# plindhorst/Ray-Tracing-Project

Measured on AMD Instinct MI355X. Metric: Mrays/s (primary) + frame ms at 1920x1080, 1M-tri BVH, 1/2/4/8 GPU, higher is better.
Workload: dtype f32; 1 GPU; C3: 1000000 random triangles (SplitMix64 seed 12345), 1920x1080 primary rays, eye (0,0,1), 1 light; frame=1920x1080, triangles=1000000, mode=primary, parallelism=tiles/1 (one GPU, whole frame), launcher=none, frames_in_flight=4, prewarm_frames=200, hw_queues=4, bvh_nodes=1145398, bvh_depth=26, ref_boxes=4480, builder=sbvh-gpu

## Files before the change

### ray-tracing-project_amd/csrc/rt_device.hip

```cpp
#include <errno.h>
#include <fcntl.h>
#include <signal.h>
#include <sys/file.h>
#include <unistd.h>

#include <atomic>
#include <cctype>
#include <chrono>
#include <condition_variable>
#include <memory>
#include <mutex>
#include <string>
#include <thread>
#include <vector>

#include "rt_dispatch.h"
#include "rt_kernels.h"

namespace rt {

constexpr int kLptBuckets = 32, kLptThreads = 512, kLptRefresh = 8;
constexpr bool kLptMoved = true;
constexpr int kLptDilate = 2;
constexpr bool kLptPred = true;
// ... 1154 lines not shown
  rt_scene::FrameSlot& slot = s->slots[slot_id];
  if ((rc = ensure_fb(slot, (size_t)fr->width * fr->height))) return rc;
  hipStream_t st = (hipStream_t)slot.stream;
  FrameParams P;
  fill_scene_params(s, P);
  fill_camera_lights(P, cam, lights, n_lights);
  P.W = fr->width, P.H = fr->height, P.tiles_x = (fr->width + 15) / 16, P.tiles_y = (fr->height + 15) / 16;
  P.shard_index = si, P.shard_count = sc, P.super_tile = frame_super_tile(sc);
  P.mode = fr->mode, P.flags = fr->flags, P.shadows = fr->mode == RT_MODE_FULL ? 1 : 0;
  P.rgb = slot.d_rgb, P.face_out = slot.d_face, P.t_out = slot.d_t, P.hits = slot.d_hits;
  P.stats = s->d_stats, P.face_boxcolor = s->d_face_boxcolor;
  if (fr->flags & RT_FRAME_STATS) {
    for (int k = 0; k < s->n_slots; k++)
      if (k != slot_id && s->slots[k].last_done) HIPCHECK(hipStreamWaitEvent(st, (hipEvent_t)s->slots[k].last_done, 0));
    HIPCHECK(hipMemsetAsync(s->d_stats, 0, kStatSlots * sizeof(unsigned long long), st));
  }
  FrameInputs in;
  in.mode = fr->mode, in.max_depth = fr->max_depth, in.flags = fr->flags;
  in.tiles_x = P.tiles_x, in.tiles_y = P.tiles_y, in.shard_index = si, in.shard_count = sc;
  in.variant = kernel_variant(), in.has_wide4 = P.sc.n_nodes4 > 0;
  in.record_bytes = (uint64_t)(s->hs.nodes.size() + s->hs.tris.size()) * 64;
  for (int k = 0; k < s->n_slots; k++)
    if (k != slot_id && s->slots[k].last_done && hipEventQuery((hipEvent_t)s->slots[k].last_done) == hipErrorNotReady)
      in.alone = false;
  in.split_k = knob_int("RT_SPLIT_K", kSplitK, 0, INT_MAX);
  in.split_kp = knob_int("RT_SPLIT_KP", kSplitKPrimary, 0, INT_MAX);
  in.timeline_split = knob_int("RT_TIMELINE_SPLIT", kKnobUnset, INT_MIN, INT_MAX) != kKnobUnset;
  const FramePlan plan = plan_frame(in);
  P.n_tiles_shard = plan.grid;
  P.max_depth = plan.depth;
  if (plan.primary_binary_tree) P.sc.wide_copy_bytes = 0;
  if (fr->flags & RT_FRAME_TIMELINE) {
    const size_t waves = in.timeline_split ? 2 * plan.units : plan.units;
    if ((rc = ensure_wave_records(slot.d_timeline, slot.timeline_waves, waves, st))) return rc;
    P.timeline = slot.d_timeline;
    s->last_timeline_waves = (int64_t)waves;
  }
  if ((fr->flags & RT_FRAME_STATS) && (fr->flags & RT_FRAME_WAVE_STATS)) {
    if (!plan.writes_wave_stats) {
      set_error("rt_render: RT_FRAME_WAVE_STATS needs the mode's own max_depth (the generic-depth kernel keeps no per-wave counts)");
      return RT_ERR_UNSUPPORTED;
    }
    const size_t lw = (size_t)plan.grid * 4;
    if ((rc = ensure_wave_records(slot.d_wave_stats, slot.wave_stats_waves, lw, st))) return rc;
    P.wave_stats = slot.d_wave_stats;
    s->last_wave_stats_waves = (int64_t)lw;
  }
  if (plan.pipeline_buffers) {
    if (sc > 1) { set_error("rt_render: the FULL stage-pipeline variant renders whole frames only"); return RT_ERR_UNSUPPORTED; }
    if ((rc = ensure_full(slot, (size_t)P.tiles_x * 16 * (size_t)P.tiles_y * 16))) return rc;
    bind_full(slot, P);
  }
  P.xcd_remap = plan.xcd_remap;
  if (plan.rotate_bands) P.xcd_rot = (int32_t)(s->band_rot++ & 7u);
  if (plan.needs_variants && !variants_linked()) {
    set_error("rt_render: kernel variant %d is an A/B build option, not in this library (make variants)", in.variant);
    return RT_ERR_UNSUPPORTED;
  }
  bool lpt_sort = false, lpt_dilated = false;
  if (plan.lpt && (rc = lpt_begin(s, plan, cam, st, P, lpt_sort, lpt_dilated))) return rc;
  if (s->ev_used + 3 > s->ev_pool.size()) {
    if (s->ev_pool.size() >= 3 * 2048) { set_error("more than 2048 renders without rt_synchronize"); return RT_ERR_INVALID; }
    for (int k = 0; k < 3; k++) {
      hipEvent_t e;
      HIPCHECK(hipEventCreate(&e));
      s->ev_pool.push_back(e);
    }
  }
  hipEvent_t* ev = (hipEvent_t*)&s->ev_pool[s->ev_used];
  s->ev_used += 3;
  HIPCHECK(hipEventRecord(ev[0], st));
  if ((rc = launch_frame(plan, s, slot, P, st, ev[1]))) return rc;
  if (lpt_sort && (rc = lpt_end(s, plan, st, lpt_dilated))) return rc;
  HIPCHECK(hipEventRecord(ev[2], st));
  slot.last_done = ev[2];
  note_frame(s, slot_id, fr, P);
  return RT_OK;
}

static int check_prefetch_word(rt_scene* s) {
#ifdef RT_CHECK_PREFETCH
  uint32_t w = 0;
  HIPCHECK(hipMemcpy(&w, s->d_pf_check, 4, hipMemcpyDeviceToHost));
  if (w) {
    set_error("RT_CHECK_PREFETCH: out-of-range scalar load offset (sites 0x%x: 0 node, 1/2 child prefetch, 3 leaf "
              "prefetch, 4 wide prefetch, 5 wide node)", w);
    return RT_ERR_HIP;
  }
#endif
  (void)s;
  return RT_OK;
}

static int sync_one(rt_scene* s, rt_stats* out) {
  int rc = check_device_scene(s);
  if (rc) return rc;
  for (int k = 0; k < s->n_slots; k++) HIPCHECK(hipStreamSynchronize((hipStream_t)s->slots[k].stream));
  if ((rc = check_prefetch_word(s))) return rc;
  struct Reset {
    rt_scene* s;
    ~Reset() {
      s->ev_used = 0;
      s->pending = false;
      for (int k = 0; k < s->n_slots; k++) s->slots[k].last_done = nullptr;
    }
  } reset_{s};
// ... 771 lines not shown
```

### ray-tracing-project_amd/csrc/rt_internal.h

```cpp
#pragma once
#include <cstdint>
#if defined(__HIPCC__) || defined(__HIP__)
#include <hip/hip_runtime.h>
#else
struct uint2 { unsigned int x, y; };
#endif

#include "rt_math.h"

namespace rt {

constexpr uint32_t kLeafBit = 0x80000000u;
constexpr uint32_t kLeafCountShift = 27;
constexpr uint32_t kLeafFirstMask = (1u << 27) - 1;
constexpr int kMaxLeaf = 16;
constexpr uint32_t kMaxFaces = (1u << 25) - 1;
constexpr int kMaxDepth = 60;
constexpr uint32_t kSafeNormalBit = 0x80000000u;
constexpr uint32_t kBoxCertBit = 0x40000000u;
constexpr uint32_t kBoxIndexMask = 0x3FFFFFFFu;

inline uint64_t record_layout(uint64_t n_nodes, uint64_t n_tris, uint64_t n_wide, uint64_t* wide_base) {
  const uint64_t bytes = (n_nodes + n_tris) * 64;
  *wide_base = 0;
  if (bytes > 0xFFFFFFFFull) return 0;
  const uint64_t wb = (bytes + 127) & ~(uint64_t)127, wide_bytes = 8 * n_wide * 128;
  if (n_wide == 0 || wb + wide_bytes > (uint64_t)kLeafBit) return bytes;
  *wide_base = wb;
  return wb + wide_bytes;
}

enum { TRAV_B2_VGPR = 0, TRAV_B2_LDS = 1, TRAV_W4 = 2, TRAV_LANE = 3 };

enum VariantBit : int {
  VB_VGPR_STACK = 1,
  VB_WIDE4 = 2,
  VB_XCD_ORDER = 4,
  VB_FULL_PIPELINE = 16,
  VB_PIPE_LANE_REFL = 32,
  VB_PIPE_LANE_SHADOW1 = 64,
  VB_PIPE_LANE_SHADOW0 = 128,
  VB_TWO_RAYS_PER_LANE = 256,
  VB_XCD_RUNS_4 = 512,
  VB_XCD_RUNS_16 = 1024,
  VB_DISPATCH_ORDER = 1536,
  VB_PERSISTENT = 2048,
  VB_PERSISTENT_NO_STEAL = 4096,
  VB_FULL_8_WAVES = 8192,
  VB_FULL_SMALL_BUILD = 16384,
  VB_SPLIT_PRIMARY = 32768,
  VB_GENERIC_DEPTH = 65536,
  VB_NO_LPT = 131072,
  VB_COARSE_COST_BUCKETS = 262144,
  VB_LPT_IN_FLIGHT = 524288,
  VB_DUAL_CHAIN = 1048576,
  VB_PRIMARY_BINARY_TREE = 2097152,
  VB_PRIMARY_UNFUSED = VB_SPLIT_PRIMARY | VB_TWO_RAYS_PER_LANE | VB_PERSISTENT,
  VB_DUAL_EXCLUDED = VB_VGPR_STACK | VB_WIDE4 | VB_XCD_ORDER | VB_PRIMARY_UNFUSED | VB_GENERIC_DEPTH,
};

// ... 105 lines not shown
};

struct FrameParams {
  DevScene sc;
  float Minv[16];
  float MS[9];
  DevMat defmat;
  float bg[3];
  float vinv[16];
  float eye[3];
  float eye_obj[3];
  float vp[4];
  float xscale, yscale;
  int32_t n_lights;
  Light lights[32];
  int32_t W, H, tiles_x, tiles_y;
  int32_t xcd_remap;
  int32_t xcd_rot;
  int32_t shard_index, shard_count, n_tiles_shard;
  int32_t super_tile;
  int32_t mode, flags;
  int32_t max_depth;
  int32_t shadows;
  float* rgb;
  int32_t* face_out;
  float* t_out;
  unsigned long long* stats;
  uint2* hits;
  HitState* state0;
  HitState* state1;
  RayRec* refl;
  uint2* hits1;
  uint32_t* blk0;
  uint32_t* blk1;
  uint32_t* list0;
  uint32_t* list1;
  uint32_t* wcount0;
  uint32_t* wcount1;
  uint32_t* woff0;
  uint32_t* woff1;
  uint32_t* counters;
  int32_t n_waves_max;
  uint32_t* timeline;
  const uint32_t* order;
  uint32_t* cost;
  uint32_t* cost_dil;
  int32_t dil_r;
  int32_t pred;
  float pred_proj[4];
  float pred_step[3];
  uint32_t* wave_stats;
  int32_t split_k;
  const float* face_boxcolor;
};

struct RayParams {
  const float* o;
  const float* d;
  int32_t n;
  int32_t* face;
  float* t;
  float* P;
  int32_t* blocked;
  float* N;
  float* rgb;
};

}
```

### ray-tracing-project_amd/csrc/rt_kernels.h

```cpp
#pragma once
#include <hip/hip_runtime.h>

#include <algorithm>
#include <atomic>
#include <cmath>
#include <cstddef>
#include <cstdio>
#include <cstring>
#include <type_traits>
#include <vector>

#include "rt_kat.h"
#include "rt_scene.h"

using rt::f3;

#define HIPCHECK(expr)                                                                   \
  do {                                                                                   \
    hipError_t e_ = (expr);                                                              \
    if (e_ != hipSuccess) {                                                              \
      rt::set_error("%s failed: %s (%s:%d)", #expr, hipGetErrorString(e_), __FILE__, __LINE__); \
      return RT_ERR_HIP;                                                                 \
    }                                                                                    \
  } while (0)
// ... 91 lines not shown
  const float dm = fmaxf(fmaxf(fabsf(r.d.x), fabsf(r.d.y)), fabsf(r.d.z));
  const bool certified = om <= kCullOriginMax && dm >= kCullDirMin && dm <= kCullDirMax;
  if (certified) {
    r.id = f3{__builtin_amdgcn_rcpf(nudge(r.d.x)), __builtin_amdgcn_rcpf(nudge(r.d.y)),
              __builtin_amdgcn_rcpf(nudge(r.d.z))};
    const float pr = kCullPadRel * om;
    const float p = pr > static_pad ? pr : 0.0f;
    r.oa = f3{-(r.o.x + p) * r.id.x, -(r.o.y + p) * r.id.y, -(r.o.z + p) * r.id.z};
    r.ob = f3{-(r.o.x - p) * r.id.x, -(r.o.y - p) * r.id.y, -(r.o.z - p) * r.id.z};
  } else {
    r.id = f3{copysignf(1.0f, nudge(r.d.x)), copysignf(1.0f, nudge(r.d.y)), copysignf(1.0f, nudge(r.d.z))};
    r.oa = f3{-r.id.x * INFINITY, -r.id.y * INFINITY, -r.id.z * INFINITY};
    r.ob = f3{r.id.x * INFINITY, r.id.y * INFINITY, r.id.z * INFINITY};
  }
}

struct Span {
  float tmin, tmax;
};
__device__ __forceinline__ Span slab(float lx, float hx, float ly, float hy, float lz, float hz, const Ray& r,
                                     float tmax_ray) {
  const float tx0 = __builtin_fmaf(lx, r.id.x, r.oa.x), tx1 = __builtin_fmaf(hx, r.id.x, r.ob.x);
  const float ty0 = __builtin_fmaf(ly, r.id.y, r.oa.y), ty1 = __builtin_fmaf(hy, r.id.y, r.ob.y);
  const float tz0 = __builtin_fmaf(lz, r.id.z, r.oa.z), tz1 = __builtin_fmaf(hz, r.id.z, r.ob.z);
  Span s;
  s.tmin = fmaxf(fmaxf(fminf(tx0, tx1), fminf(ty0, ty1)), fmaxf(fminf(tz0, tz1), 0.0f));
  s.tmax = fminf(fminf(fmaxf(tx0, tx1), fmaxf(ty0, ty1)), fminf(fmaxf(tz0, tz1), tmax_ray));
  return s;
}
template <int OCT>
__device__ __forceinline__ Span slab_o(float lx, float hx, float ly, float hy, float lz, float hz, const Ray& r,
                                       float tmax_ray) {
  if (OCT < 0) return slab(lx, hx, ly, hy, lz, hz, r, tmax_ray);
  const float nx = (OCT & 1) ? hx : lx, fx = (OCT & 1) ? lx : hx;
  const float ny = (OCT & 2) ? hy : ly, fy = (OCT & 2) ? ly : hy;
  const float nz = (OCT & 4) ? hz : lz, fz = (OCT & 4) ? lz : hz;
  const float nox = (OCT & 1) ? r.ob.x : r.oa.x, fox = (OCT & 1) ? r.oa.x : r.ob.x;
  const float noy = (OCT & 2) ? r.ob.y : r.oa.y, foy = (OCT & 2) ? r.oa.y : r.ob.y;
  const float noz = (OCT & 4) ? r.ob.z : r.oa.z, foz = (OCT & 4) ? r.oa.z : r.ob.z;
  Span s;
  s.tmin = fmaxf(fmaxf(__builtin_fmaf(nx, r.id.x, nox), __builtin_fmaf(ny, r.id.y, noy)),
                 fmaxf(__builtin_fmaf(nz, r.id.z, noz), 0.0f));
  asm("v_min3_f32 %0, %1, %2, %3\n\tv_min_f32 %0, %0, %4"
      : "=&v"(s.tmax)
      : "v"(__builtin_fmaf(fx, r.id.x, fox)), "v"(__builtin_fmaf(fy, r.id.y, foy)),
        "v"(__builtin_fmaf(fz, r.id.z, foz)), "v"(tmax_ray));
  return s;
}
constexpr int kFcmpOLE = 5;
__device__ __forceinline__ uint64_t mask_le(float a, float b) { return __builtin_amdgcn_fcmpf(a, b, kFcmpOLE); }

__device__ __forceinline__ bool ref_box_test(const DevScene& S, const Ray& r, const float* bx) {
  const float MS[9] = {S.Minv[0], S.Minv[1], S.Minv[2], S.Minv[4], S.Minv[5], S.Minv[6], S.Minv[8], S.Minv[9], S.Minv[10]};
  const f3 dd = normalized(m3v3(MS, r.d));
  const float lo[3] = {bx[0], bx[1], bx[2]}, hi[3] = {bx[4], bx[5], bx[6]};
  const float o2[3] = {r.o2.x, r.o2.y, r.o2.z}, d2[3] = {dd.x, dd.y, dd.z};
  float tin3[3], tout3[3];
#pragma unroll
  for (int k = 0; k < 3; k++) {
    const float a = (lo[k] - o2[k]) / d2[k];
    const float b = (hi[k] - o2[k]) / d2[k];
    tin3[k] = smin(a, b);
    tout3[k] = smax(a, b);
  }
  const float tin = smax(tin3[0], smax(tin3[1], tin3[2]));
  const float tout = smin(tout3[0], smin(tout3[1], tout3[2]));
  return !(tin > tout || tout < 0);
}

__device__ __forceinline__ f3 ld3(const float* p) { return f3{p[0], p[1], p[2]}; }

constexpr int kFcmpOEQ = 1, kFcmpOGE = 3, kFcmpOLT = 4, kFcmpUNE = 14, kIcmpULT = 36;
template <int PRED>
__device__ __forceinline__ uint64_t fmask(float a, float b) { return __builtin_amdgcn_fcmpf(a, b, PRED); }
__device__ __forceinline__ bool lane_in(uint64_t m) { return __builtin_amdgcn_inverse_ballot_w64(m); }

__device__ __forceinline__ uint64_t accept_candidate(const DevScene& P, const TriRec64& tr, uint32_t slot, f3 e0, f3 e2,
                                                    f3 a0, f3 a1, f3 a2, f3 p, const Ray& r, uint64_t cand) {
  if (!(tr.box & kSafeNormalBit)) {
    const float area0 = norm(a0) / 2, area1 = norm(a1) / 2, area2 = norm(a2) / 2;
    const float area = norm(cross(e0, neg(e2))) / 2;
    const float* fs = P.fshade + 12 * (size_t)slot;
    const f3 n0 = ld3(fs), n1 = ld3(fs + 4), n2 = ld3(fs + 8);
    const f3 nn = blend_normal(n0, n1, n2, area0, area1, area2, area);
    cand &= fmask<kFcmpUNE>(norm(nn), 0.0f);
  }
  if (tr.box & kBoxCertBit) {
    const float om = fmaxf(fmaxf(fabsf(r.o2.x), fabsf(r.o2.y)), fabsf(r.o2.z));
    if ((cand & ~ballot(om <= P.cert_origin_max)) == 0) return cand;
  }
  const float* bx = P.refbox + 8 * (size_t)(tr.box & kBoxIndexMask);
  const f3 X = affv3(P.Minv, p);
  const float lo[3] = {bx[0], bx[1], bx[2]}, hi[3] = {bx[4], bx[5], bx[6]};
  const float xs[3] = {X.x, X.y, X.z}, os[3] = {r.o2.x, r.o2.y, r.o2.z};
  bool inside = true;
#pragma unroll
  for (int k = 0; k < 3; k++) {
    const float m = 1e-5f * ((hi[k] - lo[k]) + fabsf(lo[k]) + fabsf(hi[k]) + fabsf(os[k])) + 1e-30f;
    inside = inside & (xs[k] > lo[k] + m) & (xs[k] < hi[k] - m);
  }
  const uint64_t ins = ballot(inside);
  if ((cand & ~ins) == 0) return cand;
  return cand & (ins | ballot(ref_box_test(P, r, bx)));
}

template <bool ANY, bool STATS = false>
__device__ __forceinline__ void test_tri(const DevScene& P, const TriRec64& tr, uint32_t slot, const Ray& r,
// ... 561 lines not shown
        switch (oct) {
          RT_WIDE_CASE(0) RT_WIDE_CASE(1) RT_WIDE_CASE(2) RT_WIDE_CASE(3)
          RT_WIDE_CASE(4) RT_WIDE_CASE(5) RT_WIDE_CASE(6) default: RT_WIDE_CASE(7)
        }
#undef RT_WIDE_CASE
      }
      if (!STATS && SL) {
        switch (oct) {
          case 0: traverse_fast<ANY, 0>(P, r, active, h, found, L.stack[wv]); return;
          case 1: traverse_fast<ANY, 1>(P, r, active, h, found, L.stack[wv]); return;
          case 2: traverse_fast<ANY, 2>(P, r, active, h, found, L.stack[wv]); return;
          case 3: traverse_fast<ANY, 3>(P, r, active, h, found, L.stack[wv]); return;
          case 4: traverse_fast<ANY, 4>(P, r, active, h, found, L.stack[wv]); return;
          case 5: traverse_fast<ANY, 5>(P, r, active, h, found, L.stack[wv]); return;
          case 6: traverse_fast<ANY, 6>(P, r, active, h, found, L.stack[wv]); return;
          default: traverse_fast<ANY, 7>(P, r, active, h, found, L.stack[wv]); return;
        }
      }
      switch (oct) {
        case 0: traverse<ANY, STATS, SL, 0>(P, r, active, h, found, L.stack[wv], cnt); return;
        case 1: traverse<ANY, STATS, SL, 1>(P, r, active, h, found, L.stack[wv], cnt); return;
        case 2: traverse<ANY, STATS, SL, 2>(P, r, active, h, found, L.stack[wv], cnt); return;
        case 3: traverse<ANY, STATS, SL, 3>(P, r, active, h, found, L.stack[wv], cnt); return;
        case 4: traverse<ANY, STATS, SL, 4>(P, r, active, h, found, L.stack[wv], cnt); return;
        case 5: traverse<ANY, STATS, SL, 5>(P, r, active, h, found, L.stack[wv], cnt); return;
        case 6: traverse<ANY, STATS, SL, 6>(P, r, active, h, found, L.stack[wv], cnt); return;
        default: traverse<ANY, STATS, SL, 7>(P, r, active, h, found, L.stack[wv], cnt); return;
      }
    }
  }
  trace<ANY, STATS, TRAV>(P, r, active, h, found, L, wv, cnt);
}
template <bool STATS, int TRAV, bool WIDE = false>
__device__ __forceinline__ void trace_closest_oct(const DevScene& P, const Ray& r, bool active, Hit& h,
                                                  WaveLds<TRAV, STATS>& L, int wv, uint32_t* cnt) {
  bool found = false;
  trace_oct<false, STATS, TRAV, WIDE, false>(P, r, active, h, found, L, wv, cnt);
}
template <bool ANY, bool STATS, int TRAV>
__device__ __forceinline__ void trace_full_ray(const DevScene& P, const Ray& r, bool active, Hit& h, bool& found,
                                               WaveLds<TRAV, STATS>& L, int wv, uint32_t* cnt) {
  trace<ANY, STATS, TRAV>(P, r, active, h, found, L, wv, cnt);
}

struct MatState {
  f3 ka, kd, ks;
  float ns;
};

__device__ __forceinline__ MatState load_mat(const DevMat& m) {
  return MatState{f3{m.ka[0], m.ka[1], m.ka[2]}, f3{m.kd[0], m.kd[1], m.kd[2]}, f3{m.ks[0], m.ks[1], m.ks[2]}, m.ns};
}

__device__ __forceinline__ f3 hit_normal(const DevScene& P, const TriRec64& tr, uint32_t slot, f3 p, int32_t& mat) {
  const f3 n{tr.nx, tr.ny, tr.nz};
  const f3 w0{tr.w0x, tr.w0y, tr.w0z}, w1{tr.w1x, tr.w1y, tr.w1z}, w2{tr.w2x, tr.w2y, tr.w2z};
  const f3 e0 = sub(w1, w0), e1 = sub(w2, w1), e2 = sub(w0, w2);
  const f3 a0 = cross(e0, sub(p, w0)), a1 = cross(e1, sub(p, w1)), a2 = cross(e2, sub(p, w2));
  const float4* fs = reinterpret_cast<const float4*>(P.fshade + 12 * (size_t)slot);
  const float4 n0 = fs[0];
  mat = __float_as_int(n0.w);
  if (dot(n, a0) < 0 || dot(n, a1) < 0 || dot(n, a2) < 0) return f3{0.0f, 0.0f, 0.0f};
  const float area0 = norm(a0) / 2, area1 = norm(a1) / 2, area2 = norm(a2) / 2;
  const float area = norm(cross(e0, neg(e2))) / 2;
  const float4 n1 = fs[1], n2 = fs[2];
  return blend_normal(f3{n0.x, n0.y, n0.z}, f3{n1.x, n1.y, n1.z}, f3{n2.x, n2.y, n2.z}, area0, area1, area2, area);
}

__device__ __forceinline__ TriRec64 vload_tri(const TriRec64* base, uint32_t i) {
  const float4* p = reinterpret_cast<const float4*>(base + i);
  TriRec64 r;
  float4* q = reinterpret_cast<float4*>(&r);
  q[0] = p[0]; q[1] = p[1]; q[2] = p[2]; q[3] = p[3];
  return r;
}


__device__ __forceinline__ Light frame_light(int l) {
  typedef const __attribute__((address_space(4))) char* KArg;
  typedef const __attribute__((address_space(4))) Light* KLight;
  const KArg base = (KArg)__builtin_amdgcn_kernarg_segment_ptr();
  const KLight q = (KLight)(base + offsetof(FrameParams, lights) + (size_t)l * sizeof(Light));
  Light r;
  for (int k = 0; k < 3; k++) {
    r.p[k] = q->p[k];
    r.c[k] = q->c[k];
  }
  r.kind = q->kind;
  return r;
}

__device__ __forceinline__ f3 light_dir(f3 p, const Light& l) {
  if (l.kind == RT_LIGHT_DIRECTIONAL) return f3{l.p[0], l.p[1], l.p[2]};
  return neg(normalized(sub(p, f3{l.p[0], l.p[1], l.p[2]})));
}

struct HitInfo {
  f3 p, n;
  int32_t mat;
  uint32_t face;
};

__device__ __forceinline__ f3 phong(const FrameParams& P, MatState& st, const HitInfo& hi, f3 o, f3 L, const float* I) {
  if (hi.mat != -1) st = load_mat(P.sc.mats[hi.mat]);
  const f3 R = phong_r(L, hi.n);
  const f3 E = normalized(sub(o, hi.p));
  const float dif = smax(dot(L, hi.n), 0.0f);
  const float spe = smax(pow_ref(dot(R, E), st.ns), 0.0f);
  return f3{(I[0] * st.ka.x + (I[0] * st.kd.x) * dif) + (I[0] * st.ks.x) * spe,
            (I[1] * st.ka.y + (I[1] * st.kd.y) * dif) + (I[1] * st.ks.y) * spe,
            (I[2] * st.ka.z + (I[2] * st.kd.z) * dif) + (I[2] * st.ks.z) * spe};
}

__device__ __forceinline__ float clamp01(float x) { return smax(smin(x, 1.0f), 0.0f); }

template <bool SHADOWS, bool STATS, int TRAV, bool OCTSH = false, bool SPLIT = false>
__device__ __forceinline__ f3 calc_color(const FrameParams& P, MatState& st, const HitInfo& hi, f3 o, bool lane_hit,
                                         WaveLds<TRAV, STATS>* lds, int wv, uint32_t* cnt) {
  f3 sum{0.0f, 0.0f, 0.0f};
  for (int l = 0; l < P.n_lights; l++) {
    const Light lt = frame_light(l);
    const f3 L = light_dir(hi.p, lt);
    bool blocked = false;
    if (SHADOWS) {
      Ray sr;
      sr.o = offset(hi.p, L, 0.003f);
      sr.d = L;
      sr.o2 = affv3(P.Minv, hi.p);
      setup_cull(sr, P.sc.static_pad);
      Hit hh{INFINITY, 0xFFFFFFFFu, 0xFFFFFFFFu};
      if (STATS && lane_hit) cnt[ST_TOTAL]++;
      if (OCTSH)
        trace_oct<true, STATS, TRAV, false, SPLIT>(P.sc, sr, lane_hit, hh, blocked, *lds, wv, cnt);
      else trace_full_ray<true, STATS, TRAV>(P.sc, sr, lane_hit, hh, blocked, *lds, wv, cnt);
    }
    f3 c{0.0f, 0.0f, 0.0f};
    if (lane_hit && !blocked) c = phong(P, st, hi, o, L, lt.c);
    sum = f3{sum.x + c.x, sum.y + c.y, sum.z + c.z};
  }
  return f3{clamp01(sum.x), clamp01(sum.y), clamp01(sum.z)};
}

struct PixelCoord {
  int px, py, wv, lane;
  int slot;
  int qw;
  int sub;
  bool active;
};

template <int WPB = 4>
__device__ __forceinline__ PixelCoord pixel_coord(const FrameParams& P) {
  PixelCoord c;
  c.lane = threadIdx.x & 63;
  int nb, b;
  int bid = (int)blockIdx.x;
  c.sub = -1;
  if (WPB == 1 && P.order != nullptr) {
    const uint32_t k = (uint32_t)P.split_k, nlog = gridDim.x - 3u * k;
    uint32_t pos = blockIdx.x;
    if (k > 0) {
      if (pos < 4u * k) {
        c.sub = (int)(pos & 3u);
        pos >>= 2;
      } else {
        pos -= 3u * k;
      }
    }
    const uint32_t o = uniform(P.order[pos]);
    bid = o < nlog ? (int)o : (int)pos;
  } else if (P.xcd_remap >= 2) {
    const int C = P.xcd_remap, G = 8 * C, full = ((int)gridDim.x / G) * G;
    if (bid < full) {
      const int x = ((bid & 7) + P.xcd_rot) & 7, k = bid >> 3;
      bid = (k / C) * G + x * C + (k % C);
    }
  }
  if (WPB == 4) {
    c.wv = (int)uniform(threadIdx.x >> 6);
    c.slot = c.wv;
    nb = (int)gridDim.x;
    b = bid;
  } else {
    c.wv = bid & 3;
    c.slot = 0;
    nb = (int)((gridDim.x - 3u * (uint32_t)P.split_k) >> 2);
    b = bid >> 2;
  }
  c.qw = b * 4 + c.wv;
  int L = b;
  if (P.xcd_remap == 1) {
    const int q = nb >> 3, rr = nb & 7, x = b & 7, k = b >> 3;
    L = x < rr ? x * (q + 1) + k : rr * (q + 1) + (x - rr) * q + k;
  }
  int tx, ty;
  shard_tile_xy(P.tiles_x, P.super_tile, P.shard_index, P.shard_count, L, tx, ty);
  c.px = tx * 16 + (c.wv & 1) * 8 + (c.lane & 7);
  c.py = ty * 16 + (c.wv >> 1) * 8 + (c.lane >> 3);
  c.active = c.px < P.W && c.py < P.H && (c.sub < 0 || (c.lane >> 4) == c.sub);
  return c;
}

__device__ __forceinline__ Ray primary_ray(const FrameParams& P, int px, int py) {
  Ray r;
  const float nx = (float)(2.0 * (double)((float)px - P.vp[0]) / (double)P.vp[2] - 1.0);
  const float ny = (float)(1.0 - 2.0 * (double)((float)py - P.vp[1]) / (double)P.vp[3]);
  const f3 w = affv3(P.vinv, f3{nx * P.xscale, ny * P.yscale, -1.0f});
  r.o = f3{P.eye[0], P.eye[1], P.eye[2]};
  r.d = normalized(sub(w, r.o));
  r.o2 = f3{P.eye_obj[0], P.eye_obj[1], P.eye_obj[2]};
  setup_cull(r, P.sc.static_pad);
  return r;
}

template <typename T>
__device__ __forceinline__ T late_kernarg(size_t off) {
  uint32_t o = (uint32_t)off;
  asm volatile("" : "+s"(o));
  typedef const __attribute__((address_space(4))) char* KArg;
  const KArg base = (KArg)__builtin_amdgcn_kernarg_segment_ptr();
  return *reinterpret_cast<const __attribute__((address_space(4))) T*>(base + o);
}

__device__ __forceinline__ void wave_clock_start(const FrameParams& P, uint32_t* clk) {
  if (P.timeline || P.cost) {
    const uint64_t t0 = __builtin_amdgcn_s_memtime();
    const uint32_t r0 = (uint32_t)__builtin_amdgcn_s_memrealtime();
    if ((threadIdx.x & 63) == 0) {
      clk[0] = (uint32_t)t0;
      clk[1] = (uint32_t)(t0 >> 32);
      clk[2] = r0;
    }
  }
}
__device__ __forceinline__ void wave_clock_end(const FrameParams& P, const uint32_t* clk, int lane, int qw,
                                               bool sub_wave = false, const float* tprim = nullptr) {
  if (!P.timeline && !P.cost) return;
  const uint64_t t1 = __builtin_amdgcn_s_memtime();
  struct { uint64_t t0; uint32_t r0; } w;
  w.t0 = (uint64_t)uniform(clk[0]) | ((uint64_t)uniform(clk[1]) << 32);
  w.r0 = uniform(clk[2]);
  if (P.cost && lane == 0) {
    const uint64_t dt = t1 - w.t0;
    const uint32_t c = dt > 0x3FFFFFFFull ? 0x3FFFFFFFu : (uint32_t)dt;
    if (!sub_wave) P.cost[qw] = c;
    else atomicMax(P.cost + qw, c);
  }
  uint32_t* const dil = late_kernarg<uint32_t*>(offsetof(FrameParams, cost_dil));
  if (dil) {
// ... 47 lines not shown
__device__ __forceinline__ void wave_stats_out(const FrameParams& P, const uint32_t* cnt, int lane, int qw, bool full) {
  if (!P.wave_stats || lane != 0) return;
  uint32_t* o = P.wave_stats + 8 * (size_t)qw;
  if (full) {
    for (int p = 0; p < 4; p++) { o[p] = cnt[ST_PS + p]; o[4 + p] = cnt[ST_PT + p]; }
  } else {
    o[0] = cnt[ST_WNODE]; o[1] = cnt[ST_WTRI]; o[2] = cnt[ST_HITS]; o[3] = 0;
    o[4] = o[5] = o[6] = o[7] = 0;
  }
}

__device__ __forceinline__ void flush_stats(const FrameParams& P, const uint32_t* cnt, int lane) {
#pragma unroll
  for (int c = 0; c < ST_COUNT; c++) {
    unsigned long long v = cnt[c];
    if (c == ST_WNODE || c == ST_WTRI || c == ST_WPOP || c == ST_WCULL || c == ST_WWIDE || c == ST_WCAND || c == ST_WPRE ||
        c == ST_WINS || c == ST_WE1 || c == ST_WE2 || c >= ST_WCANDM)
      v = (lane == 0) ? v : 0;
    for (int off = 32; off > 0; off >>= 1) v += __shfl_xor(v, off, 64);
    if (lane == 0 && v) atomicAdd(P.stats + c, v);
  }
}


constexpr int kTraceWavesPerEu = 8;
constexpr int kTraceWPB = 1;
template <bool STATS, int TRAV>
__global__ __launch_bounds__(64 * kTraceWPB) __attribute__((amdgpu_waves_per_eu(kTraceWavesPerEu)))
void k_trace_primary(FrameParams P) {
  __shared__ WaveLds<TRAV, STATS> lds;
  const PixelCoord c = pixel_coord<kTraceWPB>(P);
  uint32_t cnt[ST_COUNT] = {};
  const Ray r = primary_ray(P, c.px, c.py);
  if (STATS && c.active) { cnt[ST_RAYS]++; cnt[ST_TOTAL]++; }
  Hit h{INFINITY, 0xFFFFFFFFu, 0xFFFFFFFFu};
  trace_closest_oct<STATS, TRAV, true>(P.sc, r, c.active, h, lds, c.slot, cnt);
  if (STATS && c.active && h.t != INFINITY) cnt[ST_HITS]++;
  if (c.active) P.hits[(size_t)c.py * P.W + c.px] = make_uint2(__float_as_uint(h.t), h.slot);
  if (P.wcount0 != nullptr) {
    const uint32_t nh = (uint32_t)__popcll(ballot(c.active && h.t != INFINITY));
    if (c.lane == 0) P.wcount0[c.qw] = nh;
  }
  if (STATS) {
    if (P.wave_stats) {
      uint32_t w[ST_COUNT];
      for (int k = 0; k < ST_COUNT; k++) w[k] = cnt[k];
      w[ST_HITS] = (uint32_t)__popcll(ballot(c.active && h.t != INFINITY));
      wave_stats_out(P, w, c.lane, c.qw, false);
    }
    flush_stats(P, cnt, c.lane);
  }
}

template <bool HITS, bool BOXCOL = false>
__device__ __forceinline__ void shade_primary_pixel(const FrameParams& P, const Ray& r, size_t pix, float t,
                                                    uint32_t slot) {
  const bool hit0 = t != INFINITY;
  f3 col;
  int32_t face = -1;
  if (BOXCOL && hit0) {
    face = (int32_t)P.sc.tris[slot].face;
    const float4 c = reinterpret_cast<const float4*>(P.face_boxcolor)[face];
    col = f3{c.x, c.y, c.z};
  } else if (hit0) {
    const TriRec64 tr0 = vload_tri(P.sc.tris, slot);
    HitInfo hi0;
    hi0.face = tr0.face;
    face = (int32_t)tr0.face;
    hi0.p = f3{r.o.x + t * r.d.x, r.o.y + t * r.d.y, r.o.z + t * r.d.z};
    hi0.n = hit_normal(P.sc, tr0, slot, hi0.p, hi0.mat);
    MatState st = load_mat(P.defmat);
    const f3 direct0 = calc_color<false, false, TRAV_B2_LDS>(P, st, hi0, r.o, true, nullptr, 0, nullptr);
    if (hi0.mat != -1) st.ks = load_mat(P.sc.mats[hi0.mat]).ks;
    col = f3{clamp01(direct0.x + 0.0f * st.ks.x), clamp01(direct0.y + 0.0f * st.ks.y),
             clamp01(direct0.z + 0.0f * st.ks.z)};
  } else {
    col = f3{P.bg[0], P.bg[1], P.bg[2]};
  }
  P.rgb[3 * pix + 0] = col.x;
  P.rgb[3 * pix + 1] = col.y;
  P.rgb[3 * pix + 2] = col.z;
  if (HITS) {
    P.face_out[pix] = face;
    P.t_out[pix] = t;
  }
}

template <bool HITS, bool BOXCOL>
__global__ __launch_bounds__(256) void k_shade_primary(FrameParams P) {
  const PixelCoord c = pixel_coord(P);
  if (!c.active) return;
  const size_t pix = (size_t)c.py * P.W + c.px;
  const uint2 hb = P.hits[pix];
  const float t = __uint_as_float(hb.x);
  Ray r;
  if (t != INFINITY) r = primary_ray(P, c.px, c.py);
  shade_primary_pixel<HITS, BOXCOL>(P, r, pix, t, hb.y);
}


template <bool HITS, bool BOXCOL = false>
__global__ __launch_bounds__(64 * kTraceWPB) __attribute__((amdgpu_waves_per_eu(kTraceWavesPerEu)))
void k_primary_fused(FrameParams P) {
  __shared__ WaveLds<TRAV_B2_LDS, false> lds;
  __shared__ float tprim[64];
  wave_clock_start(P, lds.clk);
  const PixelCoord c = pixel_coord<kTraceWPB>(P);
  Ray r = primary_ray(P, c.px, c.py);
  asm("" : "+v"(r.o.x), "+v"(r.o.y), "+v"(r.o.z));
  Hit h{INFINITY, 0xFFFFFFFFu, 0xFFFFFFFFu};
  trace_closest_oct<false, TRAV_B2_LDS, true>(P.sc, r, c.active, h, lds, c.slot, nullptr);
  tprim[c.lane] = h.t;
  if (c.active) shade_primary_pixel<HITS, BOXCOL>(P, r, (size_t)c.py * P.W + c.px, h.t, h.slot);
  wave_clock_end(P, lds.clk, c.lane, c.qw, c.sub >= 0, tprim);
}

struct PhaseMark {
  uint32_t n0, t0;
};
template <bool STATS>
__device__ __forceinline__ PhaseMark phase_begin(const uint32_t* cnt) {
  if (!STATS) return PhaseMark{0, 0};
  return PhaseMark{cnt[ST_WNODE], cnt[ST_WTRI]};
}
template <bool STATS>
__device__ __forceinline__ void phase_end(uint32_t* cnt, int p, const PhaseMark& m, bool act) {
  if (!STATS) return;
  const uint64_t b = ballot(act);
// ... 316 lines not shown
```

Baseline: 10260 Mrays/s.

## Use fast integer division for tile mapping and uniform material loads in primary shading

Replaces the integer divisions in the block-to-tile mapping with precomputed multiply-shift divisors computed on the host and passed in FrameParams, and adds a range check on the block and tile counts. Primary shading now loads the shade record before the triangle, computes the blended normal branch-free, and detects wave-uniform materials through ballot/readlane so the material is read once through the constant address space instead of per lane and per light. An asm barrier is added in ref_box_test to pin the ray direction in registers. The changes cut integer ALU and redundant memory traffic in the shading and tile-index paths, at the cost of a larger FrameParams and more special-case code.

```diff
diff --git a/ray-tracing-project_amd/csrc/rt_device.hip b/ray-tracing-project_amd/csrc/rt_device.hip
--- a/ray-tracing-project_amd/csrc/rt_device.hip
+++ b/ray-tracing-project_amd/csrc/rt_device.hip
@@ -1230,6 +1230,16 @@
     bind_full(slot, P);
   }
   P.xcd_remap = plan.xcd_remap;
+  {
+    const uint64_t S2 = (uint64_t)P.super_tile * P.super_tile;
+    const uint64_t blocks = (uint64_t)plan.units + 3ull * (uint64_t)plan.split_ceiling;
+    const uint64_t tiles = ((uint64_t)plan.grid + S2) * (uint64_t)sc + (uint64_t)si;
+    if (!fastdiv_in_range(blocks) || !fastdiv_in_range(tiles)) {
+      set_error("rt_render: the frame has more blocks than the tile arithmetic covers (2^31)");
+      return RT_ERR_INVALID;
+    }
+    P.div = make_tile_divs(P.xcd_remap, P.tiles_x, P.super_tile);
+  }
   if (plan.rotate_bands) P.xcd_rot = (int32_t)(s->band_rot++ & 7u);
   if (plan.needs_variants && !variants_linked()) {
     set_error("rt_render: kernel variant %d is an A/B build option, not in this library (make variants)", in.variant);
diff --git a/ray-tracing-project_amd/csrc/rt_fastdiv.h b/ray-tracing-project_amd/csrc/rt_fastdiv.h
--- /dev/null
+++ b/ray-tracing-project_amd/csrc/rt_fastdiv.h
@@ -0,0 +1,88 @@
+#pragma once
+#include <cstdint>
+
+#if defined(__HIPCC__) || defined(__HIP__)
+#define RT_FD_HD __host__ __device__ inline
+#else
+#define RT_FD_HD inline
+#endif
+
+namespace rt {
+
+struct FastDiv {
+  uint32_t mul, shift;
+};
+
+constexpr uint32_t kFastDivLimit = 0x80000000u;
+RT_FD_HD bool fastdiv_in_range(uint64_t n) { return n < kFastDivLimit; }
+
+inline FastDiv make_fastdiv(uint32_t d) {
+  if (d == 0 || d >= kFastDivLimit) d = 1;
+  uint32_t l = 0;
+  while ((1ull << l) < d) l++;
+  const uint64_t p = 1ull << (31 + l);
+  return FastDiv{(uint32_t)((p + d - 1) / d), l};
+}
+
+RT_FD_HD uint32_t fd_mulhi(uint32_t a, uint32_t b) {
+#if defined(__HIP_DEVICE_COMPILE__)
+  return __umulhi(a, b);
+#else
+  return (uint32_t)(((uint64_t)a * b) >> 32);
+#endif
+}
+RT_FD_HD uint32_t fd_div(uint32_t n, FastDiv f) { return fd_mulhi(n << 1, f.mul) >> f.shift; }
+RT_FD_HD void fd_divmod(uint32_t n, FastDiv f, uint32_t d, uint32_t& q, uint32_t& r) {
+  q = fd_div(n, f);
+  r = n - q * d;
+}
+
+struct TileDivs {
+  FastDiv run;
+  FastDiv group;
+  FastDiv tiles_x;
+  FastDiv super2;
+  FastDiv super;
+  FastDiv super_row;
+  uint32_t super_row_n;
+};
+inline TileDivs make_tile_divs(int xcd_remap, int tiles_x, int S) {
+  TileDivs t;
+  const uint32_t C = xcd_remap >= 1 ? (uint32_t)xcd_remap : 1u, s = S >= 1 ? (uint32_t)S : 1u;
+  const uint32_t tx = tiles_x >= 1 ? (uint32_t)tiles_x : 1u;
+  t.run = make_fastdiv(C);
+  t.group = make_fastdiv(8 * C);
+  t.tiles_x = make_fastdiv(tx);
+  t.super2 = make_fastdiv(s * s);
+  t.super = make_fastdiv(s);
+  t.super_row_n = (tx + s - 1) / s;
+  t.super_row = make_fastdiv(t.super_row_n);
+  return t;
+}
+
+RT_FD_HD int xcd_chunk_block(const TileDivs& D, int C, int rot, uint32_t grid, int bid) {
+  const int G = 8 * C, full = (int)fd_div(grid, D.group) * G;
+  if (bid >= full) return bid;
+  const int x = ((bid & 7) + rot) & 7;
+  uint32_t kq, kr;
+  fd_divmod((uint32_t)bid >> 3, D.run, (uint32_t)C, kq, kr);
+  return (int)kq * G + x * C + (int)kr;
+}
+
+RT_FD_HD void shard_tile_xy_fd(const TileDivs& D, int tiles_x, int S, int index, int count, int L, int& tx, int& ty) {
+  uint32_t q, r;
+  if (S <= 1) {
+    fd_divmod((uint32_t)(index + L * count), D.tiles_x, (uint32_t)tiles_x, q, r);
+    tx = (int)r;
+    ty = (int)q;
+    return;
+  }
+  uint32_t j, k, kq, kr;
+  fd_divmod((uint32_t)L, D.super2, (uint32_t)(S * S), j, k);
+  fd_divmod((uint32_t)index + j * (uint32_t)count, D.super_row, D.super_row_n, q, r);
+  fd_divmod(k, D.super, (uint32_t)S, kq, kr);
+  tx = (int)(r * (uint32_t)S + kr);
+  ty = (int)(q * (uint32_t)S + kq);
+}
+
+}
diff --git a/ray-tracing-project_amd/csrc/rt_internal.h b/ray-tracing-project_amd/csrc/rt_internal.h
--- a/ray-tracing-project_amd/csrc/rt_internal.h
+++ b/ray-tracing-project_amd/csrc/rt_internal.h
@@ -6,6 +6,7 @@
 struct uint2 { unsigned int x, y; };
 #endif
 
+#include "rt_fastdiv.h"
 #include "rt_math.h"
 
 namespace rt {
@@ -217,6 +218,7 @@
   uint32_t* wave_stats;
   int32_t split_k;
   const float* face_boxcolor;
+  TileDivs div;
 };
 
 struct RayParams {
diff --git a/ray-tracing-project_amd/csrc/rt_kernels.h b/ray-tracing-project_amd/csrc/rt_kernels.h
--- a/ray-tracing-project_amd/csrc/rt_kernels.h
+++ b/ray-tracing-project_amd/csrc/rt_kernels.h
@@ -167,7 +167,9 @@
 
 __device__ __forceinline__ bool ref_box_test(const DevScene& S, const Ray& r, const float* bx) {
   const float MS[9] = {S.Minv[0], S.Minv[1], S.Minv[2], S.Minv[4], S.Minv[5], S.Minv[6], S.Minv[8], S.Minv[9], S.Minv[10]};
-  const f3 dd = normalized(m3v3(MS, r.d));
+  f3 d = r.d;
+  asm volatile("" : "+v"(d.x), "+v"(d.y), "+v"(d.z));
+  const f3 dd = normalized(m3v3(MS, d));
   const float lo[3] = {bx[0], bx[1], bx[2]}, hi[3] = {bx[4], bx[5], bx[6]};
   const float o2[3] = {r.o2.x, r.o2.y, r.o2.z}, d2[3] = {dd.x, dd.y, dd.z};
   float tin3[3], tout3[3];
@@ -835,19 +837,36 @@
   return MatState{f3{m.ka[0], m.ka[1], m.ka[2]}, f3{m.kd[0], m.kd[1], m.kd[2]}, f3{m.ks[0], m.ks[1], m.ks[2]}, m.ns};
 }
 
-__device__ __forceinline__ f3 hit_normal(const DevScene& P, const TriRec64& tr, uint32_t slot, f3 p, int32_t& mat) {
+struct ShadeRec {
+  float4 n0, n1, n2;
+};
+__device__ __forceinline__ ShadeRec load_shade(const DevScene& P, uint32_t slot) {
+  const float4* fs = reinterpret_cast<const float4*>(P.fshade + 12 * (size_t)slot);
+  return ShadeRec{fs[0], fs[1], fs[2]};
+}
+__device__ __forceinline__ int32_t shade_mat(const ShadeRec& s) { return __float_as_int(s.n0.w); }
+__device__ __forceinline__ f3 hit_normal(const TriRec64& tr, const ShadeRec& s, f3 p) {
   const f3 n{tr.nx, tr.ny, tr.nz};
   const f3 w0{tr.w0x, tr.w0y, tr.w0z}, w1{tr.w1x, tr.w1y, tr.w1z}, w2{tr.w2x, tr.w2y, tr.w2z};
   const f3 e0 = sub(w1, w0), e1 = sub(w2, w1), e2 = sub(w0, w2);
   const f3 a0 = cross(e0, sub(p, w0)), a1 = cross(e1, sub(p, w1)), a2 = cross(e2, sub(p, w2));
-  const float4* fs = reinterpret_cast<const float4*>(P.fshade + 12 * (size_t)slot);
-  const float4 n0 = fs[0];
-  mat = __float_as_int(n0.w);
-  if (dot(n, a0) < 0 || dot(n, a1) < 0 || dot(n, a2) < 0) return f3{0.0f, 0.0f, 0.0f};
+  const bool outside = dot(n, a0) < 0 || dot(n, a1) < 0 || dot(n, a2) < 0;
   const float area0 = norm(a0) / 2, area1 = norm(a1) / 2, area2 = norm(a2) / 2;
   const float area = norm(cross(e0, neg(e2))) / 2;
-  const float4 n1 = fs[1], n2 = fs[2];
-  return blend_normal(f3{n0.x, n0.y, n0.z}, f3{n1.x, n1.y, n1.z}, f3{n2.x, n2.y, n2.z}, area0, area1, area2, area);
+  const f3 b = blend_normal(f3{s.n0.x, s.n0.y, s.n0.z}, f3{s.n1.x, s.n1.y, s.n1.z}, f3{s.n2.x, s.n2.y, s.n2.z}, area0, area1,
+                            area2, area);
+  return f3{outside ? 0.0f : b.x, outside ? 0.0f : b.y, outside ? 0.0f : b.z};
+}
+__device__ __forceinline__ f3 hit_normal(const DevScene& P, const TriRec64& tr, uint32_t slot, f3 p, int32_t& mat) {
+  const ShadeRec s = load_shade(P, slot);
+  mat = shade_mat(s);
+  return hit_normal(tr, s, p);
+}
+
+__device__ __forceinline__ MatState load_mat_uniform(const DevMat* mats, int32_t id) {
+  typedef const __attribute__((address_space(4))) DevMat* KMat;
+  const KMat q = (KMat)(uintptr_t)(mats + id);
+  return MatState{f3{q->ka[0], q->ka[1], q->ka[2]}, f3{q->kd[0], q->kd[1], q->kd[2]}, f3{q->ks[0], q->ks[1], q->ks[2]}, q->ns};
 }
 
 __device__ __forceinline__ TriRec64 vload_tri(const TriRec64* base, uint32_t i) {
@@ -884,8 +903,7 @@
   uint32_t face;
 };
 
-__device__ __forceinline__ f3 phong(const FrameParams& P, MatState& st, const HitInfo& hi, f3 o, f3 L, const float* I) {
-  if (hi.mat != -1) st = load_mat(P.sc.mats[hi.mat]);
+__device__ __forceinline__ f3 phong_state(const MatState& st, const HitInfo& hi, f3 o, f3 L, const float* I) {
   const f3 R = phong_r(L, hi.n);
   const f3 E = normalized(sub(o, hi.p));
   const float dif = smax(dot(L, hi.n), 0.0f);
@@ -894,12 +912,17 @@
             (I[1] * st.ka.y + (I[1] * st.kd.y) * dif) + (I[1] * st.ks.y) * spe,
             (I[2] * st.ka.z + (I[2] * st.kd.z) * dif) + (I[2] * st.ks.z) * spe};
 }
+__device__ __forceinline__ f3 phong(const FrameParams& P, MatState& st, const HitInfo& hi, f3 o, f3 L, const float* I) {
+  if (hi.mat != -1) st = load_mat(P.sc.mats[hi.mat]);
+  return phong_state(st, hi, o, L, I);
+}
 
 __device__ __forceinline__ float clamp01(float x) { return smax(smin(x, 1.0f), 0.0f); }
 
 template <bool SHADOWS, bool STATS, int TRAV, bool OCTSH = false, bool SPLIT = false>
 __device__ __forceinline__ f3 calc_color(const FrameParams& P, MatState& st, const HitInfo& hi, f3 o, bool lane_hit,
-                                         WaveLds<TRAV, STATS>* lds, int wv, uint32_t* cnt) {
+                                         WaveLds<TRAV, STATS>* lds, int wv, uint32_t* cnt, bool st_ready = false) {
+  const bool once = !SHADOWS && st_ready;
   f3 sum{0.0f, 0.0f, 0.0f};
   for (int l = 0; l < P.n_lights; l++) {
     const Light lt = frame_light(l);
@@ -918,7 +941,7 @@
       else trace_full_ray<true, STATS, TRAV>(P.sc, sr, lane_hit, hh, blocked, *lds, wv, cnt);
     }
     f3 c{0.0f, 0.0f, 0.0f};
-    if (lane_hit && !blocked) c = phong(P, st, hi, o, L, lt.c);
+    if (lane_hit && !blocked) c = once ? phong_state(st, hi, o, L, lt.c) : phong(P, st, hi, o, L, lt.c);
     sum = f3{sum.x + c.x, sum.y + c.y, sum.z + c.z};
   }
   return f3{clamp01(sum.x), clamp01(sum.y), clamp01(sum.z)};
@@ -953,11 +976,7 @@
     const uint32_t o = uniform(P.order[pos]);
     bid = o < nlog ? (int)o : (int)pos;
   } else if (P.xcd_remap >= 2) {
-    const int C = P.xcd_remap, G = 8 * C, full = ((int)gridDim.x / G) * G;
-    if (bid < full) {
-      const int x = ((bid & 7) + P.xcd_rot) & 7, k = bid >> 3;
-      bid = (k / C) * G + x * C + (k % C);
-    }
+    bid = xcd_chunk_block(P.div, P.xcd_remap, P.xcd_rot, gridDim.x, bid);
   }
   if (WPB == 4) {
     c.wv = (int)uniform(threadIdx.x >> 6);
@@ -977,7 +996,7 @@
     L = x < rr ? x * (q + 1) + k : rr * (q + 1) + (x - rr) * q + k;
   }
   int tx, ty;
-  shard_tile_xy(P.tiles_x, P.super_tile, P.shard_index, P.shard_count, L, tx, ty);
+  shard_tile_xy_fd(P.div, P.tiles_x, P.super_tile, P.shard_index, P.shard_count, L, tx, ty);
   c.px = tx * 16 + (c.wv & 1) * 8 + (c.lane & 7);
   c.py = ty * 16 + (c.wv >> 1) * 8 + (c.lane >> 3);
   c.active = c.px < P.W && c.py < P.H && (c.sub < 0 || (c.lane >> 4) == c.sub);
@@ -1131,6 +1150,26 @@
   }
 }
 
+__device__ __forceinline__ f3 shade_primary_hit(const FrameParams& P, const Ray& r, float t, const TriRec64& tr0,
+                                                const ShadeRec& sr0) {
+  HitInfo hi0;
+  hi0.mat = shade_mat(sr0);
+  const uint64_t hits = ballot(true), with = ballot(hi0.mat != -1);
+  const int32_t m0 = with != 0 ? __builtin_amdgcn_readlane(hi0.mat, (int)__builtin_ctzll(with)) : 0;
+  const bool uniform_mat = with == 0 || (with == hits && ballot(hi0.mat != m0) == 0);
+  MatState st = load_mat(P.defmat);
+  if (uniform_mat) {
+    if (with != 0) st = load_mat_uniform(P.sc.mats, m0);
+  } else if (hi0.mat != -1) {
+    st = load_mat(P.sc.mats[hi0.mat]);
+  }
+  hi0.face = tr0.face;
+  hi0.p = f3{r.o.x + t * r.d.x, r.o.y + t * r.d.y, r.o.z + t * r.d.z};
+  hi0.n = hit_normal(tr0, sr0, hi0.p);
+  const f3 direct0 = calc_color<false, false, TRAV_B2_LDS>(P, st, hi0, r.o, true, nullptr, 0, nullptr, true);
+  return f3{clamp01(direct0.x + 0.0f * st.ks.x), clamp01(direct0.y + 0.0f * st.ks.y), clamp01(direct0.z + 0.0f * st.ks.z)};
+}
+
 template <bool HITS, bool BOXCOL = false>
 __device__ __forceinline__ void shade_primary_pixel(const FrameParams& P, const Ray& r, size_t pix, float t,
                                                     uint32_t slot) {
@@ -1142,17 +1181,10 @@
     const float4 c = reinterpret_cast<const float4*>(P.face_boxcolor)[face];
     col = f3{c.x, c.y, c.z};
   } else if (hit0) {
+    const ShadeRec sr0 = load_shade(P.sc, slot);
     const TriRec64 tr0 = vload_tri(P.sc.tris, slot);
-    HitInfo hi0;
-    hi0.face = tr0.face;
     face = (int32_t)tr0.face;
-    hi0.p = f3{r.o.x + t * r.d.x, r.o.y + t * r.d.y, r.o.z + t * r.d.z};
-    hi0.n = hit_normal(P.sc, tr0, slot, hi0.p, hi0.mat);
-    MatState st = load_mat(P.defmat);
-    const f3 direct0 = calc_color<false, false, TRAV_B2_LDS>(P, st, hi0, r.o, true, nullptr, 0, nullptr);
-    if (hi0.mat != -1) st.ks = load_mat(P.sc.mats[hi0.mat]).ks;
-    col = f3{clamp01(direct0.x + 0.0f * st.ks.x), clamp01(direct0.y + 0.0f * st.ks.y),
-             clamp01(direct0.z + 0.0f * st.ks.z)};
+    col = shade_primary_hit(P, r, t, tr0, sr0);
   } else {
     col = f3{P.bg[0], P.bg[1], P.bg[2]};
   }
```

New measurement: 10250 Mrays/s, median of 2. Within noise of the previous version (-0.2%).
